# COx2/docker-nvidia-glx-desktop

Measured on AMD Instinct MI355X. Metric: encoded FPS + p50 end-to-end latency at 1080p60 H.264; concurrent sessions/node, higher is better.
Workload: dtype uint8 video (8-bit 4:2:0), H.264 Constrained Baseline

## Files before the change

csrc/bindings/module.cpp:

```cpp
#include <pybind11/numpy.h>
#include <pybind11/pybind11.h>
#include <pybind11/stl.h>

#include <cstring>

#include "../codec/h264_core.h"
#include "../codec/h264_encoder.h"
#include "../codec/vp8_encoder.h"
#include "../codec/hevc_encoder.h"
#include "../common/hip_check.h"
#include "../common/trace.h"
#include "../kernels/pixel.h"
#include "../runtime/session.h"

namespace py = pybind11;
using namespace mx;

void register_net(py::module& m);
void register_audio(py::module& m);
void register_rfb(py::module& m);

namespace {

template <class T>
T* as_ptr(uintptr_t p) {
    return reinterpret_cast<T*>(p);
}
hipStream_t as_stream(uintptr_t s) { return reinterpret_cast<hipStream_t>(s); }

py::bytes to_bytes(const std::vector<uint8_t>& v) {
    return py::bytes(reinterpret_cast<const char*>(v.data()), v.size());
}

struct PyBits {
    std::vector<uint32_t> words;
    h264::BitWriter w;
    PyBits() : words(4096) { w.init(words.data()); }
    py::tuple finish() {
        const uint32_t bits = w.bits;
        w.flush();
        std::vector<uint8_t> out;
        for (uint32_t i = 0; i < (bits + 7) / 8; ++i) out.push_back((uint8_t)(words[i / 4] >> (24 - 8 * (i % 4))));
        return py::make_tuple(to_bytes(out), bits);
    }
};

py::tuple cavlc_block_py(const std::vector<int>& coef, int nc) {
    PyBits b;
    int16_t c[16] = {0};
    const int n = (int)coef.size();
    if (n != 4 && n != 15 && n != 16) throw std::invalid_argument("block must have 4, 15 or 16 coefficients");
    for (int i = 0; i < n; ++i) c[i] = (int16_t)coef[i];
    h264::cavlc_block(b.w, c, n, nc);
    return b.finish();
}

py::array_t<int> fdct_py(py::array_t<int, py::array::c_style | py::array::forcecast> x) {
    if (x.size() != 16) throw std::invalid_argument("need 16 values");
    py::array_t<int> y(16);
    h264::fdct4x4(x.data(), y.mutable_data());
    return y;
}
py::array_t<int> idct_py(py::array_t<int, py::array::c_style | py::array::forcecast> x) {
    if (x.size() != 16) throw std::invalid_argument("need 16 values");
    py::array_t<int> y(16);
    h264::idct4x4(x.data(), y.mutable_data());
    return y;
}

py::array_t<uint8_t> copy_plane(const uint8_t* dev, int pitch, int w, int h) {
    py::array_t<uint8_t> out({h, w});
    HIP_CHECK(hipDeviceSynchronize());
    HIP_CHECK(hipMemcpy2D(out.mutable_data(), w, dev, pitch, w, h, hipMemcpyDeviceToHost));
    return out;
}

}

PYBIND11_MODULE(_native, m) {
    m.doc() = "mxdesk native runtime: HIP kernels (gfx950), H.264 encoder, session pipeline";

    m.def("device_count", []() {
        int n = 0;
        if (hipGetDeviceCount(&n) != hipSuccess) return 0;
        return n;
    });
    m.def("set_device", [](int d) { HIP_CHECK(hipSetDevice(d)); });
    m.def("device_name", [](int d) {
        hipDeviceProp_t p;
        HIP_CHECK(hipGetDeviceProperties(&p, d));
        return std::string(p.gcnArchName) + " / " + p.name;
    });
    m.def("synchronize", []() { HIP_CHECK(hipDeviceSynchronize()); });
    register_net(m);
    register_audio(m);
    register_rfb(m);
    m.def("now_us", &Session::now_us, "CLOCK_MONOTONIC microseconds (same clock as time.monotonic())");

    py::module h = m.def_submodule("h264", "H.264 building blocks (for tests)");
    h.def("hpel_planes", [](py::array_t<uint8_t, py::array::c_style> ref, int coded_w) {
        if (ref.ndim() != 2 || coded_w % 16 || ref.shape(0) % 16 || ref.shape(1) < coded_w)
            throw std::invalid_argument("ref must be (coded_h, pitch) with 16-aligned coded size");
        int hp = 0;
        auto planes = h264::hpel_planes_for_test(ref.data(), coded_w, (int)ref.shape(0), (int)ref.shape(1), &hp);
        const int rows = (int)ref.shape(0) + 2 * h264::kHpelPad;
        py::list out;
        for (auto& p : planes) {
            py::array_t<uint8_t> a({rows, hp});
            std::memcpy(a.mutable_data(), p.data(), p.size());
            out.append(a);
        }
        return out;
    });
    h.def("mc_luma_gpu", [](py::array_t<uint8_t, py::array::c_style> ref, int coded_w, int x4, int y4) {
        if (ref.ndim() != 2 || coded_w % 16 || ref.shape(0) % 16 || ref.shape(1) < coded_w)
            throw std::invalid_argument("ref must be (coded_h, pitch) with 16-aligned coded size");
        py::array_t<uint8_t> out({16, 16});
        h264::mc_luma_for_test(ref.data(), coded_w, (int)ref.shape(0), (int)ref.shape(1), x4, y4, out.mutable_data());
        return out;
    }, py::arg("ref"), py::arg("coded_w"), py::arg("x4"), py::arg("y4"),
          "16x16 luma prediction at quarter-sample position (x4, y4) by k_inter_encode's interpolation");
    h.def("cavlc_block", &cavlc_block_py, py::arg("coef"), py::arg("nc"));
    h.def("fdct4x4", &fdct_py);
    h.def("idct4x4", &idct_py);
    h.def("ue", [](uint32_t k) {
        PyBits b;
        h264::put_ue(b.w, k);
        return b.finish();
    });
    h.def("se", [](int v) {
        PyBits b;
        h264::put_se(b.w, v);
        return b.finish();
    });
    h.def("luma_qpel", [](py::array_t<uint8_t, py::array::c_style> plane, int x4, int y4) {
        if (plane.ndim() != 2) throw std::invalid_argument("2-D plane");
        const int H = (int)plane.shape(0), W = (int)plane.shape(1);
        return h264::luma_qpel(plane.data(), W, W, H, x4, y4);
    });
    h.def("level_for", &h264::pick_level);
    h.def("zero_sum_4x4", [](int qp) { return h264::zero_sum_4x4(qp); }, py::arg("qp"));
    h.def("zero_sum_chroma_dc", [](int qpc) { return h264::zero_sum_chroma_dc(qpc); }, py::arg("qpc"));
    h.def("chroma_qp", [](int qp, int offset) { return h264::chroma_qp(qp, offset); }, py::arg("qp"),
          py::arg("offset") = 0);
    h.def("quant4x4", [](py::array_t<int, py::array::c_style | py::array::forcecast> y, int qp, bool intra, int start) {
        if (y.size() != 16) throw std::invalid_argument("need 16 values");
        py::array_t<int> z(16);
        const int nz = h264::quant4x4(y.data(), z.mutable_data(), qp, intra, start);
        return py::make_tuple(z, nz);
    }, py::arg("y"), py::arg("qp"), py::arg("intra") = false, py::arg("start") = 0);
    h.def("quant_dc_chroma", [](py::array_t<int, py::array::c_style | py::array::forcecast> dc, int qpc, bool intra) {
        if (dc.size() != 4) throw std::invalid_argument("need 4 values");
        py::array_t<int> z(4);
        const int nz = h264::quant_dc_chroma(dc.data(), z.mutable_data(), qpc, intra);
        return py::make_tuple(z, nz);
    }, py::arg("dc"), py::arg("qpc"), py::arg("intra") = false);
    h.def("luma_block_inter", [](py::array_t<int, py::array::c_style | py::array::forcecast> res, int qp) {
        if (res.size() != 16) throw std::invalid_argument("need 16 values");
        py::array_t<int> z(16), rr(16);
        const int nz = h264::luma_block_inter(res.data(), qp, z.mutable_data(), rr.mutable_data());
        return py::make_tuple(z, rr, nz);
    }, py::arg("res"), py::arg("qp"), "inter luma block: residual (raster) -> levels (scan), reconstructed residual, nz");

    py::class_<h264::EncoderConfig>(m, "EncoderConfig")
        .def(py::init<>())
        .def_readwrite("width", &h264::EncoderConfig::width)
        .def_readwrite("height", &h264::EncoderConfig::height)
        .def_readwrite("fps", &h264::EncoderConfig::fps)
        .def_readwrite("bitrate_kbps", &h264::EncoderConfig::bitrate_kbps)
        .def_readwrite("qp", &h264::EncoderConfig::qp)
        .def_readwrite("qp_min", &h264::EncoderConfig::qp_min)
        .def_readwrite("qp_max", &h264::EncoderConfig::qp_max)
        .def_readwrite("keyint", &h264::EncoderConfig::keyint)
        .def_readwrite("search_range", &h264::EncoderConfig::search_range)
        .def_readwrite("scroll_range", &h264::EncoderConfig::scroll_range)
        .def_readwrite("me_coarse", &h264::EncoderConfig::me_coarse)
        .def_readwrite("intra4x4", &h264::EncoderConfig::intra4x4)
        .def_readwrite("subpel", &h264::EncoderConfig::subpel)
        .def_readwrite("chroma_qp_offset", &h264::EncoderConfig::chroma_qp_offset)
        .def_readwrite("pipeline_depth", &h264::EncoderConfig::pipeline_depth)
        .def_readwrite("aq", &h264::EncoderConfig::aq)
        .def_readwrite("intra_in_p", &h264::EncoderConfig::intra_in_p)
        .def_readwrite("vp8_bpred", &h264::EncoderConfig::vp8_bpred)
        .def_readwrite("vp8_intra", &h264::EncoderConfig::vp8_intra)
        .def_readwrite("mask_x0", &h264::EncoderConfig::mask_x0)
        .def_readwrite("mask_y0", &h264::EncoderConfig::mask_y0)
        .def_readwrite("mask_x1", &h264::EncoderConfig::mask_x1)
        .def_readwrite("mask_y1", &h264::EncoderConfig::mask_y1)
        .def_readwrite("deblock", &h264::EncoderConfig::deblock)
        .def_readwrite("partitions", &h264::EncoderConfig::partitions)
        .def_readwrite("tu_split", &h264::EncoderConfig::tu_split)
        .def_readwrite("hevc_slice_cost", &h264::EncoderConfig::hevc_slice_cost)
        .def_readwrite("hevc_wpp", &h264::EncoderConfig::hevc_wpp)
        .def_readwrite("hevc_wpp_rows", &h264::EncoderConfig::hevc_wpp_rows)
        .def_readwrite("sao", &h264::EncoderConfig::sao)
        .def_readwrite("hevc_chroma_keep", &h264::EncoderConfig::hevc_chroma_keep)
        .def_readwrite("hevc_intra_split", &h264::EncoderConfig::hevc_intra_split);

    py::class_<h264::FrameStats>(m, "FrameStats")
        .def_readonly("frame_index", &h264::FrameStats::frame_index)
        .def_readonly("idr", &h264::FrameStats::idr)
        .def_readonly("qp", &h264::FrameStats::qp)
        .def_readonly("bytes", &h264::FrameStats::bytes)
        .def_readonly("skipped_mbs", &h264::FrameStats::skipped_mbs)
        .def_readonly("encode_ms", &h264::FrameStats::encode_ms)
// ... 715 lines not shown
```

csrc/codec/h264_core.h:

```cpp
#pragma once
#include <hip/hip_runtime.h>
#include <stdint.h>

#include "h264_tables.h"

#define MXHD __host__ __device__ __forceinline__

namespace mx {
namespace h264 {

struct BitWriter {
    uint32_t* words;
    uint32_t nwords;
    uint64_t acc;
    int nacc;
    uint32_t bits;

    MXHD void init(uint32_t* w) {
        words = w;
        nwords = 0;
        acc = 0;
        nacc = 0;
        bits = 0;
    }
// ... 207 lines not shown
    if (nC < 8) return 2;
    return 3;
}

template <class W>
MXHD int cavlc_block(W& w, const int16_t* coef, int maxNum, int nC) {
    int total = 0, last = -1, t1 = 0;
    bool t1_open = true;
    for (int i = maxNum - 1; i >= 0; --i) {
        const int c = coef[i];
        if (c != 0) {
            if (last < 0) last = i;
            if (t1_open) {
                if ((c == 1 || c == -1) && t1 < 3) ++t1;
                else t1_open = false;
            }
            ++total;
        }
    }
    const int tab = nc_table(nC);
    if (total == 0) {
        w.put(kCoeffToken0[tab].code, kCoeffToken0[tab].len);
        return 0;
    }
    const Vlc ct = kCoeffToken[tab][total - 1][t1];
    w.put(ct.code, ct.len);
    int sl = (total > 10 && t1 < 3) ? 1 : 0;
    int k = 0;
    for (int i = last; i >= 0; --i) {
        const int l = coef[i];
        if (l == 0) continue;
        if (k < t1) {
            w.put(l < 0 ? 1u : 0u, 1);
            ++k;
            continue;
        }
        int code = l > 0 ? 2 * l - 2 : -2 * l - 1;
        if (k == t1 && t1 < 3) code -= 2;
        if (sl == 0) {
            if (code < 14) {
                w.put(1, code + 1);
            } else if (code < 30) {
                w.put(1, 15);
                w.put(code - 14, 4);
            } else {
                w.put(1, 16);
                w.put(code - 30, 12);
            }
        } else {
            if (code < (15 << sl)) {
                w.put(1, (code >> sl) + 1);
                w.put(code & ((1 << sl) - 1), sl);
            } else {
                w.put(1, 16);
                w.put(code - (15 << sl), 12);
            }
        }
        if (sl == 0) sl = 1;
        const int a = l < 0 ? -l : l;
        if (a > (3 << (sl - 1)) && sl < 6) ++sl;
        ++k;
    }
    const int total_zeros = last + 1 - total;
    if (total < maxNum) {
        const Vlc tz = (maxNum == 4) ? kTotalZerosDc[total - 1][total_zeros] : kTotalZeros[total - 1][total_zeros];
        w.put(tz.code, tz.len);
    }
    int zl = total_zeros;
    int i = last;
    for (int seen = 0; seen < total - 1 && zl > 0; ++seen) {
        int j = i - 1, rb = 0;
        while (coef[j] == 0) {
            ++rb;
            --j;
        }
        const Vlc v = kRunBefore[(zl > 7 ? 7 : zl) - 1][rb];
        w.put(v.code, v.len);
        zl -= rb;
        i = j;
    }
    return total;
}

struct SeqParams {
    int width, height;
    int mb_w, mb_h;
    int level_idc;
    int log2_max_frame_num;
    int fps_num, fps_den;
};

MXHD int pick_level(int mbs, int fps) {
    long mbps = (long)mbs * fps;
    if (mbs <= 1620 && mbps <= 40500) return 30;
    if (mbs <= 3600 && mbps <= 108000) return 31;
    if (mbs <= 5120 && mbps <= 216000) return 32;
    if (mbs <= 8192 && mbps <= 245760) return 40;
    if (mbs <= 8704 && mbps <= 522240) return 42;
    if (mbs <= 22080 && mbps <= 589824) return 50;
    if (mbs <= 36864 && mbps <= 983040) return 51;
    if (mbs <= 36864) return 52;
    if (mbs <= 139264 && mbps <= 4177920) return 60;
    if (mbs <= 139264 && mbps <= 8355840) return 61;
    return 62;
}

template <class W>
MXHD void write_sps(W& w, const SeqParams& p) {
    w.put(66, 8);
    w.put(0xC0, 8);
    w.put(p.level_idc, 8);
    put_ue(w, 0);
    put_ue(w, p.log2_max_frame_num - 4);
    put_ue(w, 2);
    put_ue(w, 1);
    w.put(0, 1);
    put_ue(w, p.mb_w - 1);
    put_ue(w, p.mb_h - 1);
    w.put(1, 1);
    w.put(1, 1);
    const int crop_r = (p.mb_w * 16 - p.width) / 2, crop_b = (p.mb_h * 16 - p.height) / 2;
    if (crop_r || crop_b) {
        w.put(1, 1);
        put_ue(w, 0);
        put_ue(w, crop_r);
        put_ue(w, 0);
        put_ue(w, crop_b);
    } else {
        w.put(0, 1);
    }
    w.put(1, 1);
    w.put(0, 1);
    w.put(0, 1);
    w.put(1, 1);
    w.put(5, 3);
    w.put(0, 1);
    w.put(1, 1);
    w.put(1, 8);
    w.put(1, 8);
    w.put(1, 8);
    w.put(0, 1);
    w.put(1, 1);
    w.put((uint32_t)p.fps_den, 32);
    w.put((uint32_t)(2 * p.fps_num), 32);
    w.put(0, 1);
    w.put(0, 1);
    w.put(0, 1);
    w.put(0, 1);
    w.put(1, 1);
    w.put(1, 1);
    put_ue(w, 0);
    put_ue(w, 0);
    put_ue(w, 16);
    put_ue(w, 16);
    put_ue(w, 0);
    put_ue(w, 1);
    w.put(1, 1);
    w.flush();
}

template <class W>
MXHD void write_pps(W& w, int init_qp, int chroma_qp_offset) {
    put_ue(w, 0);
    put_ue(w, 0);
    w.put(0, 1);
    w.put(0, 1);
// ... 177 lines not shown
```

csrc/codec/h264_kernels.hip:

```cpp
#include <hip/hip_runtime.h>

#include <cstddef>

#include "../common/hip_check.h"
#include "../common/wave.h"
#include "h264_core.h"
#include "h264_deblock.h"
#include "h264_gpu.h"
#include "h264_mb.h"

namespace mx {
namespace h264 {

namespace {

__device__ __forceinline__ uint32_t bswap32(uint32_t v) { return __builtin_bswap32(v); }

constexpr int kHpTW = 128, kHpTH = 16;
constexpr int kHpSW = kHpTW + 8;
__device__ __forceinline__ int byte_of(uint32_t w, int k) { return (int)((w >> (8 * k)) & 0xff); }
__device__ __forceinline__ uint32_t pack4(int a, int b, int c, int d) {
    const uint32_t lo = __builtin_amdgcn_perm((uint32_t)b, (uint32_t)a, 0x0c0c0400u);
    const uint32_t hi = __builtin_amdgcn_perm((uint32_t)d, (uint32_t)c, 0x0c0c0400u);
    return __builtin_amdgcn_perm(hi, lo, 0x05040100u);
// ... 2092 lines not shown
        intra_luma_mb(g, f, ls, m, mc, mbx, mby, av, lt, ldc, lane, s0);
        const int r = lane >> 2, c4 = (lane & 3) * 4;
        const uint32_t v = (uint32_t)lt[1 + r][1 + c4] | ((uint32_t)lt[1 + r][2 + c4] << 8) |
                           ((uint32_t)lt[1 + r][3 + c4] << 16) | ((uint32_t)lt[1 + r][4 + c4] << 24);
        *reinterpret_cast<uint32_t*>(fs->rec_y + (y0 + r) * g.pitch + x0 + c4) = v;
    } else {
        const int xc0 = mbx * 8, yc0 = mby * 8;
        if (lane < 32) {
            const int r = lane >> 2, c4 = (lane & 3) * 4;
            cs[lane] = *reinterpret_cast<const uint32_t*>(src_uv + (size_t)(yc0 + r) * g.pitch + mbx * 16 + c4);
        }
        if (lane < 16) {
            const int comp = lane >> 3, r = lane & 7;
            ct[comp][1 + r][0] = av.left ? fs->rec_uv[(yc0 + r) * g.pitch + 2 * (xc0 - 1) + comp] : 0;
        } else if (lane < 34) {
            const int k = lane - 16, comp = k / 9, cx = k - comp * 9;
            const bool ok = cx == 0 ? av.topleft : av.top;
            ct[comp][0][cx] = ok ? fs->rec_uv[(yc0 - 1) * g.pitch + 2 * (xc0 - 1 + cx) + comp] : 0;
        }
        wave_lds_sync();
        intra_chroma_mb(g, fs->chroma_qp_offset, f, cs, m, mc, mbx, mby, av, ct, cdc, lane, s0, s1);
        if (lane < 32) {
            const int r = lane >> 2, c2 = (lane & 3) * 2;
            const uint32_t v = (uint32_t)ct[0][1 + r][1 + c2] | ((uint32_t)ct[1][1 + r][1 + c2] << 8) |
                               ((uint32_t)ct[0][1 + r][2 + c2] << 16) | ((uint32_t)ct[1][1 + r][2 + c2] << 24);
            *reinterpret_cast<uint32_t*>(fs->rec_uv + (yc0 + r) * g.pitch + 2 * (xc0 + c2)) = v;
        }
    }
    unsigned long long a = s0, b = s1;
    for (int o = 32; o > 0; o >>= 1) {
        a += __shfl_xor(a, o, 64);
        b += __shfl_xor(b, o, 64);
    }
    __syncthreads();
    const int nmb = g.mb_w * g.mb_h;
    const int slot = mby;
    if (lane == 0) {
        if (wave == 0) {
            m.cbp = (uint8_t)((m.cbp & 15) | (m.cbp_c << 4));
            atomicAdd(&fs->sse_part[slot], a - mb_sse[mbi]);
            if (mb_unmasked(fs, mbx, mby)) atomicAdd(&fs->sse_part[3 * kSsePartStride + slot], a - mb_sse[mbi]);
        } else {
            atomicAdd(&fs->sse_part[kSsePartStride + slot], a - mb_sse[nmb + mbi]);
            atomicAdd(&fs->sse_part[2 * kSsePartStride + slot], b - mb_sse[2 * nmb + mbi]);
        }
    }
}

__global__ __launch_bounds__(128) void k_intra_p(Geometry g, const FrameState* __restrict__ fs,
                                                 const uint8_t* __restrict__ src_y, const uint8_t* __restrict__ src_uv,
                                                 MbInfo* __restrict__ mbs, int16_t* __restrict__ coef,
                                                 const int32_t* __restrict__ gain, const uint32_t* __restrict__ mb_sse,
                                                 const int* __restrict__ wave_prog, const int* __restrict__ cand) {
    const int ncand = wave_prog[1];
    for (int k = blockIdx.x; k < ncand; k += gridDim.x) intra_p_mb(g, fs, src_y, src_uv, mbs, coef, gain, mb_sse, cand[k]);
}

__device__ __forceinline__ uint32_t mask_bits(int n) { return n >= 32 ? 0xffffffffu : ((1u << n) - 1); }

template <class F>
__device__ __forceinline__ void overlap(uint32_t& acc, uint32_t W0, uint32_t s0, uint32_t len, F getbits) {
    const uint32_t lo = max(W0, s0), hi = min(W0 + 32, s0 + len);
    if (lo >= hi) return;
    const int n = (int)(hi - lo);
    const uint32_t bits = getbits(lo - s0, n) & mask_bits(n);
    acc |= bits << (W0 + 32 - hi);
}

constexpr int kRoleWords = 24;
__device__ __forceinline__ uint32_t role_get(const uint32_t* buf, uint32_t b, int n) {
    const uint32_t wi = b >> 5, sh = b & 31;
    const uint64_t hi = ((uint64_t)buf[wi] << 32) | (wi + 1 < (uint32_t)kRoleWords ? buf[wi + 1] : 0u);
    return (uint32_t)((hi << sh) >> (64 - n));
}

constexpr int kCavlcMbPerBlock = 8;
template <bool kQuad>
__global__ __launch_bounds__(256) void k_cavlc(Geometry g, const FrameState* __restrict__ fs, MbInfo* __restrict__ mbs,
                                               const int16_t* __restrict__ coef, uint32_t* __restrict__ slot,
                                               uint32_t* __restrict__ slot_bits) {
    static_assert(kNumRoles < 32, "the roles of one MB (plus the total slot) must fit a half-wave");
    __shared__ uint32_t rbuf[kCavlcMbPerBlock][kNumRoles][kRoleWords];
    __shared__ uint32_t roff[kCavlcMbPerBlock][kNumRoles + 1];
    __shared__ __attribute__((aligned(16))) int16_t cbuf[kCavlcMbPerBlock][kCoefStride];
    __shared__ MbInfo nbuf[kCavlcMbPerBlock][5];
    static_assert(sizeof(MbInfo) % 4 == 0, "MbInfo copied as dwords");
    const int hw = (threadIdx.x >> 5) & 1, lane = threadIdx.x & 31;
    const int wave = threadIdx.x >> 5;
    const int nmb = g.mb_w * g.mb_h;
    const int mbi = blockIdx.x * kCavlcMbPerBlock + wave;
    if (mbi >= nmb) return;
    const int mbx = mbi % g.mb_w, mby = mbi / g.mb_w;
    const Avail av = mb_avail(g, mbx, mby, fs->slice_rows);
    {
        const int src[5] = {mbi, mbi - 1, mbi - g.mb_w, mbi - g.mb_w + 1, mbi - g.mb_w - 1};
        const bool ok[5] = {true, av.left, av.top, av.topright, av.topleft};
        constexpr int kW = (int)(sizeof(MbInfo) / 4);
        for (int q = lane; q < 5 * kW; q += 32) {
            const int k = q / kW, d = q - k * kW;
            if (ok[k]) reinterpret_cast<uint32_t*>(&nbuf[wave][k])[d] = reinterpret_cast<const uint32_t*>(&mbs[src[k]])[d];
        }
        wave_lds_sync();
    }
    const MbNbrs nb{&nbuf[wave][0], &nbuf[wave][1], &nbuf[wave][2], &nbuf[wave][3], &nbuf[wave][4]};
    const MbInfo& m = nbuf[wave][0];
    const int16_t* mc = coef + (size_t)mbi * kCoefStride;

    int mvd[kQuad ? 8 : 4];
    const bool skip = decide_skip<kQuad>(nb, av, mvd);
    int dqp = 0;
    if (!skip && !fs->idr && carries_dqp(m)) {
        const int per_slice = fs->slice_rows * g.mb_w, first = (mbi / per_slice) * per_slice;
        int pred = fs->qp;
        bool found = false;
        constexpr int kPer = 16;
        for (int j0 = mbi - 1; j0 >= first && !found; j0 -= 32 * kPer) {
            int qv[kPer];
#pragma unroll
            for (int k = 0; k < kPer; ++k) {
                const int j = j0 - 32 * k - lane;
                qv[k] = -1;
                if (j >= first) {
                    const MbInfo& mj = mbs[j];
                    if (carries_dqp(mj)) qv[k] = mj.qp;
                }
            }
#pragma unroll
            for (int k = 0; k < kPer; ++k) {
                const unsigned long long bal = __ballot(qv[k] >= 0);
                const uint32_t hb = (uint32_t)(bal >> (32 * hw));
                const int q = __shfl(qv[k], hb ? (int)(__ffs(hb) - 1) : 0, 32);
                if (!found && hb) {
                    pred = q;
                    found = true;
                }
            }
        }
        dqp = qp_delta(m.qp, pred);
    }
    if (!skip) {
        const uint4* src = reinterpret_cast<const uint4*>(mc);
        uint4* dst = reinterpret_cast<uint4*>(cbuf[wave]);
        for (int q = lane; q < kCoefStride / 8; q += 32) dst[q] = src[q];
    }
    wave_lds_sync();
    uint32_t bits = 0;
    if (!skip && lane < kNumRoles) {
        BitWriter w;
        w.init(rbuf[wave][lane]);
        code_role<kQuad>(w, lane, g, fs->idr, nb, cbuf[wave], av, mvd, dqp);
        w.flush();
        bits = w.bits;
    }
    uint32_t incl = bits;
    incl += (uint32_t)__builtin_amdgcn_update_dpp(0, (int)incl, 0x111, 0xF, 0xF, false);
    incl += (uint32_t)__builtin_amdgcn_update_dpp(0, (int)incl, 0x112, 0xF, 0xF, false);
    incl += (uint32_t)__builtin_amdgcn_update_dpp(0, (int)incl, 0x114, 0xF, 0xF, false);
    incl += (uint32_t)__builtin_amdgcn_update_dpp(0, (int)incl, 0x118, 0xF, 0xF, false);
    incl += (uint32_t)__builtin_amdgcn_update_dpp(0, (int)incl, 0x142, 0xA, 0xF, false);
    const uint32_t total = __shfl(incl, 31, 32);
    if (lane < kNumRoles) roff[wave][lane] = incl - bits;
    if (lane == kNumRoles) roff[wave][kNumRoles] = total;
    wave_lds_sync();
    const bool fits = total <= kSlotWords * 32u;
    if (!skip && fits) {
        const uint32_t nwords = (total + 31) >> 5;
        uint32_t* dst = slot + (size_t)mbi * kSlotWords;
        for (uint32_t wi = lane; wi < nwords; wi += 32) {
            const uint32_t W0 = wi * 32;
            int r = 0;
            while (r < kNumRoles - 1 && roff[wave][r + 1] <= W0) ++r;
            uint32_t acc = 0;
            for (; r < kNumRoles; ++r) {
                const uint32_t o = roff[wave][r], len = roff[wave][r + 1] - o;
                if (o >= W0 + 32) break;
                if (len == 0) continue;
                overlap(acc, W0, o, len, [&](uint32_t x, int n) { return role_get(rbuf[wave][r], x, n); });
            }
            dst[wi] = acc;
        }
    }
    if (lane == 0) {
        slot_bits[mbi] = skip ? 0u : (fits ? total : 0xffffffffu);
        mbs[mbi].skip = skip ? 1 : 0;
    }
}

constexpr int kScanThreads = 256;
constexpr int kScanRowPer = 2;
constexpr int kScanMaxRows = 512;

__device__ __forceinline__ uint32_t blk_excl_sum(uint32_t v, uint32_t* wbuf, uint32_t* total) {
    return blk_excl_scan<kScanThreads, uint32_t>(v, 0u, [](uint32_t a, uint32_t b) { return a + b; }, wbuf, total);
}
__device__ __forceinline__ int blk_excl_max(int v, int init, int* wbuf, int* total) {
    return blk_excl_scan<kScanThreads, int>(v, init, [](int a, int b) { return max(a, b); }, wbuf, total);
}

__device__ __forceinline__ SliceParams slice_params(const FrameState* fs, int s, int mb_w) {
    return make_slice_params(s * fs->slice_rows * mb_w, fs->idr, fs->frame_num, fs->log2_max_frame_num,
                             fs->idr_pic_id, fs->qp - fs->pic_init_qp, fs->deblock_off);
}

template <bool kQuad>
__global__ __launch_bounds__(kScanThreads) void k_scan_rows(Geometry g, const FrameState* __restrict__ fs,
                                                            const uint32_t* __restrict__ slot_bits,
                                                            uint4* __restrict__ row_agg,
                                                            unsigned long long* __restrict__ row_sse,
                                                            const MbInfo* __restrict__ mbs, uint32_t* __restrict__ db_cnt,
                                                            const uint32_t* __restrict__ mb_sse) {
    __shared__ int wi[kScanThreads / 64];
    __shared__ uint32_t wu[kScanThreads / 64];
    const int t = threadIdx.x, r = blockIdx.x, base = r * g.mb_w;
    const bool idr = fs->idr != 0;
    const int nmb = g.mb_w * g.mb_h;
    const bool per_mb = !idr && fs->deblock_off;
    unsigned long long acc[4] = {0, 0, 0, 0};
    if (per_mb) {
        for (int j = t; j < g.mb_w; j += kScanThreads) {
            const uint32_t sy = mb_sse[base + j];
            acc[0] += sy;
            acc[1] += mb_sse[nmb + base + j];
            acc[2] += mb_sse[2 * nmb + base + j];
            acc[3] += mb_unmasked(fs, j, r) ? sy : 0u;
        }
    }
    if (t == 0 && (!per_mb || fs->intra_in_p))
        for (int c = 0; c < 4; ++c) acc[c] += fs->sse_part[c * kSsePartStride + r];
    uint32_t b[kScanRowPer];
    int last = -1, first = 0x7fffffff;
    uint32_t ncoded = 0, over = 0;
#pragma unroll
    for (int k = 0; k < kScanRowPer; ++k) {
// ... 501 lines not shown
```

csrc/codec/h264_mb.h:

```cpp
#pragma once
#include "h264_core.h"
#include "h264_gpu.h"
#include "h264_intra.h"

namespace mx {
namespace h264 {

constexpr int kNumRoles = 28;

struct Avail {
    bool left, top, topright, topleft;
};

MXHD Avail mb_avail(const Geometry& g, int mbx, int mby, int slice_rows) {
    Avail a;
    const bool top_same_slice = mby > 0 && (mby / slice_rows) == ((mby - 1) / slice_rows);
    a.left = mbx > 0;
    a.top = top_same_slice;
    a.topright = top_same_slice && mbx < g.mb_w - 1;
    a.topleft = top_same_slice && mbx > 0;
    return a;
}

MXHD int combine_nc(bool ha, int na, bool hb, int nb) {
// ... 73 lines not shown
            c = mv_nb_blk<kQuad>(nb.left, av.left, 3, 1);
            if (a.ref == 0) return a.mv;
        }
    } else {
        if (idx == 0) {
            a = mv_nb_blk<kQuad>(nb.left, av.left, 3, 0);
            b = mv_nb_blk<kQuad>(nb.top, av.top, 0, 3);
            c = av.top ? mv_nb_blk<kQuad>(nb.top, true, 2, 3) : mv_nb_blk<kQuad>(nb.topleft, av.topleft, 3, 3);
            if (a.ref == 0) return a.mv;
        } else {
            a = own;
            b = mv_nb_blk<kQuad>(nb.top, av.top, 2, 3);
            c = av.topright ? mv_nb_blk<kQuad>(nb.topright, true, 0, 3) : mv_nb_blk<kQuad>(nb.top, av.top, 1, 3);
            if (c.ref == 0) return c.mv;
        }
    }
    return predict_mv16x16(a, b, c);
}

MXHD Mv predict_mv_quad(const MbNbrs& nb, const Avail& av, int q) {
    auto own = [&](int k) {
        MvNb n;
        n.avail = true;
        n.ref = 0;
        n.mv = quad_mv(*nb.self, k);
        return n;
    };
    MvNb a, b, c;
    if (q == 0) {
        a = mv_nb_blk(nb.left, av.left, 3, 0);
        b = mv_nb_blk(nb.top, av.top, 0, 3);
        c = av.top ? mv_nb_blk(nb.top, true, 2, 3) : mv_nb_blk(nb.topleft, av.topleft, 3, 3);
    } else if (q == 1) {
        a = own(0);
        b = mv_nb_blk(nb.top, av.top, 2, 3);
        c = av.topright ? mv_nb_blk(nb.topright, true, 0, 3) : mv_nb_blk(nb.top, av.top, 1, 3);
    } else if (q == 2) {
        a = mv_nb_blk(nb.left, av.left, 3, 2);
        b = own(0);
        c = own(1);
    } else {
        a = own(2);
        b = own(1);
        c = own(0);
    }
    return predict_mv16x16(a, b, c);
}

template <bool kQuad = true>
MXHD bool decide_skip(const MbNbrs& nb, const Avail& av, int* mvd) {
    const MbInfo& m = *nb.self;
    mvd[0] = mvd[1] = mvd[2] = mvd[3] = 0;
    if (kQuad) mvd[4] = mvd[5] = mvd[6] = mvd[7] = 0;
    if (m.type != kMbP16x16) return false;
    if (kQuad && m.part == kPart8x8) {
        for (int q = 0; q < 4; ++q) {
            const Mv v = quad_mv(m, q), p = predict_mv_quad(nb, av, q);
            mvd[2 * q] = v.x - p.x;
            mvd[2 * q + 1] = v.y - p.y;
        }
        return false;
    }
    if (m.part != kPart16x16) {
        const Mv v0{m.pmv[0], m.pmv[1]}, v1{m.pmv[2], m.pmv[3]};
        const Mv p0 = predict_mv_part<kQuad>(nb, av, m.part, 0, v0);
        const Mv p1 = predict_mv_part<kQuad>(nb, av, m.part, 1, v0);
        mvd[0] = v0.x - p0.x;
        mvd[1] = v0.y - p0.y;
        mvd[2] = v1.x - p1.x;
        mvd[3] = v1.y - p1.y;
        return false;
    }
    const MvNb a = mv_nb_blk<kQuad>(nb.left, av.left, 3, 0);
    const MvNb b = mv_nb_blk<kQuad>(nb.top, av.top, 0, 3);
    MvNb c = mv_nb_blk<kQuad>(nb.topright, av.topright, 0, 3);
    if (!av.topright) c = mv_nb_blk<kQuad>(nb.topleft, av.topleft, 3, 3);
    const Mv pskip = predict_mv_skip(a, b, c);
    const Mv p = predict_mv16x16(a, b, c);
    mvd[0] = m.mvx - p.x;
    mvd[1] = m.mvy - p.y;
    return m.cbp == 0 && m.mvx == pskip.x && m.mvy == pskip.y;
}

template <bool kQuad = true, class W>
MXHD void code_role(W& w, int role, const Geometry& g, int idr, const MbNbrs& nb, const int16_t* mc,
                    const Avail& av, const int* mvd, int dqp = 0) {
    const MbInfo& m = *nb.self;
    const bool intra = m.type == kMbI16x16;
    const int cbp = m.cbp;
    const int cbp_l = cbp & 15, cbp_c = cbp >> 4;
    const MbInfo* ml = av.left ? nb.left : nullptr;
    const MbInfo* mt = av.top ? nb.top : nullptr;
    if (role == 0) {
        if (intra) {
            const int mbtype = 1 + m.i16_mode + 4 * cbp_c + (cbp_l ? 12 : 0);
            put_ue(w, (uint32_t)(idr ? mbtype : 5 + mbtype));
            put_ue(w, m.chroma_mode);
            put_se(w, dqp);
        } else if (m.type == kMbI4x4) {
            put_ue(w, idr ? 0u : 5u);
            for (int b = 0; b < 16; ++b) {
                const int bx = kBlkX[b], by = kBlkY[b];
                const bool ha = bx > 0 || av.left, hb = by > 0 || av.top;
                int ma = -1, mb = -1;
                if (bx > 0) ma = i4_get(m.i4, by * 4 + bx - 1);
                else if (ml && ml->type == kMbI4x4) ma = i4_get(ml->i4, by * 4 + 3);
                if (by > 0) mb = i4_get(m.i4, (by - 1) * 4 + bx);
                else if (mt && mt->type == kMbI4x4) mb = i4_get(mt->i4, 12 + bx);
                const int pm = i4_pred_mode(ma, mb, ha, hb);
                const int mode = i4_get(m.i4, by * 4 + bx);
                if (mode == pm) {
                    w.put(1, 1);
                } else {
                    w.put(0, 1);
                    w.put((uint32_t)(mode < pm ? mode : mode - 1), 3);
                }
            }
            put_ue(w, m.chroma_mode);
            put_ue(w, (uint32_t)cbp_to_codenum(cbp, true));
            if (cbp) put_se(w, dqp);
        } else {
            put_ue(w, m.part);
            if (kQuad && m.part == kPart8x8)
                for (int q = 0; q < 4; ++q) put_ue(w, 0u);
            put_se(w, mvd[0]);
            put_se(w, mvd[1]);
            if (m.part != kPart16x16) {
                put_se(w, mvd[2]);
                put_se(w, mvd[3]);
            }
            if (kQuad && m.part == kPart8x8)
                for (int i = 4; i < 8; ++i) put_se(w, mvd[i]);
            put_ue(w, (uint32_t)cbp_to_codenum(cbp, false));
            if (cbp) put_se(w, dqp);
        }
        return;
    }
    if (role == 1) {
        if (!intra) return;
        const int nc = combine_nc(av.left, ml ? ml->nz_luma[3] : 0, av.top, mt ? mt->nz_luma[12] : 0);
        cavlc_block(w, mc + kCoefLumaDc, 16, nc);
        return;
    }
    if (role <= 17) {
        const int b = role - 2;
        if (!(cbp_l & (1 << (b >> 2)))) return;
        const int bx = kBlkX[b], by = kBlkY[b];
        const bool ha = bx > 0 || av.left, hb = by > 0 || av.top;
        const int na = bx > 0 ? m.nz_luma[by * 4 + bx - 1] : (ml ? ml->nz_luma[by * 4 + 3] : 0);
        const int nb = by > 0 ? m.nz_luma[(by - 1) * 4 + bx] : (mt ? mt->nz_luma[12 + bx] : 0);
        const int nc = combine_nc(ha, na, hb, nb);
        if (intra) {
            cavlc_block(w, mc + kCoefLuma + b * 16 + 1, 15, nc);
        } else {
            cavlc_block(w, mc + kCoefLuma + b * 16, 16, nc);
        }
        return;
    }
    if (role <= 19) {
        if (!cbp_c) return;
        const int comp = role - 18;
        cavlc_block(w, mc + kCoefChromaDc + comp * 4, 4, -1);
        return;
    }
    if (role < kNumRoles) {
        if (cbp_c != 2) return;
        const int comp = (role - 20) >> 2, cb = (role - 20) & 3, bx = cb & 1, by = cb >> 1;
        const uint8_t* own = comp ? m.nz_cr : m.nz_cb;
        const uint8_t* lft = ml ? (comp ? ml->nz_cr : ml->nz_cb) : nullptr;
        const uint8_t* top = mt ? (comp ? mt->nz_cr : mt->nz_cb) : nullptr;
        const bool ha = bx > 0 || av.left, hb = by > 0 || av.top;
        const int na = bx > 0 ? own[by * 2] : (lft ? lft[by * 2 + 1] : 0);
        const int nb = by > 0 ? own[bx] : (top ? top[2 + bx] : 0);
        const int nc = combine_nc(ha, na, hb, nb);
        cavlc_block(w, mc + kCoefChromaAc + (comp * 4 + cb) * 16 + 1, 15, nc);
    }
}

MXHD int aq_mb_qp(int frame_qp, uint32_t sad, int aq) {
    if (!aq) return frame_qp;
    const int off = sad > 256u * 48 ? 12 : (sad > 256u * 32 ? 6 : 0);
    const int q = frame_qp + off;
    return q > 51 ? 51 : q;
}

MXHD int lambda_sse(int qp) {
    constexpr int tab[52] = {0,   0,   0,   0,   0,   0,   0,   0,   0,    0,    1,    1,    1,    1,
                             1,   2,   2,   3,   3,   4,   5,   7,   9,    11,   14,   17,   22,   27,
                             34,  43,  54,  69,  86,  109, 137, 173, 218,  274,  345,  435,  548,  691,
                             870, 1097, 1382, 1741, 2193, 2763, 3482, 4387, 5527, 6963};
    return tab[qp < 0 ? 0 : (qp > 51 ? 51 : qp)];
}
MXHD uint32_t block_bits_est(int nz) { return nz ? 2u + 6u * (uint32_t)nz : 0u; }
MXHD bool drop_residual(int aq, uint32_t lsad, int qp, long long d_pred, long long d_coded, uint32_t bits) {
    if (aq < 2 || lsad <= 256u * 32) return false;
    return d_pred - d_coded < (long long)lambda_sse(qp) * (long long)bits;
}

constexpr uint32_t kTsadChanging = 256u * 24, kTsadPersistent = 256u * 2;
constexpr int kAqChangingOffset = 6, kAqPersistentOffset = -6;
MXHD int aq_static_offset(int aq) { return kAqPersistentOffset - 3 * ((aq > 6 ? 6 : aq) - 3); }
enum TClass : int { kTcNormal = 0, kTcPersistent = 1, kTcChanging = 2, kTcStatic = 3 };
MXHD int temporal_class(uint32_t tsad, bool zero_mv) {
    return tsad > kTsadChanging ? kTcChanging
                                : (tsad == 0 && zero_mv ? kTcStatic : (tsad <= kTsadPersistent ? kTcPersistent : kTcNormal));
}
MXHD int aq3_mb_qp(int frame_qp, int tclass, int aq = 3) {
    const int q = frame_qp + (tclass == kTcChanging     ? kAqChangingOffset
                              : tclass == kTcStatic     ? aq_static_offset(aq)
                              : tclass == kTcPersistent ? kAqPersistentOffset
                                                        : 0);
    return q < 0 ? 0 : (q > 51 ? 51 : q);
}
MXHD int mb_qp_for(int frame_qp, uint32_t lsad, int tclass, int aq) {
    return aq >= 3 ? aq3_mb_qp(frame_qp, tclass, aq) : aq_mb_qp(frame_qp, lsad, aq);
}
MXHD bool drop_luma_for(int aq, uint32_t lsad, int tclass, int qp, long long d_pred, long long d_coded,
                        uint32_t bits) {
    if (aq >= 3)
        return tclass == kTcChanging && d_pred - d_coded < (long long)lambda_sse(qp) * (long long)bits;
    return drop_residual(aq, lsad, qp, d_pred, d_coded, bits);
}
MXHD bool drop_luma_possible(int aq, uint32_t lsad, int tclass) {
    return aq >= 3 ? tclass == kTcChanging : (aq >= 2 && lsad > 256u * 32);
}
MXHD bool drop_chroma_for(int aq, int tclass, bool luma_dropped) {
    return luma_dropped || (aq >= 3 && tclass == kTcChanging);
}

MXHD uint32_t inter_cost(uint32_t satd, int frame_qp, int mvx, int mvy) {
    return satd + (uint32_t)(lambda_sad(frame_qp) * (mvd_bits(mvx) + mvd_bits(mvy)));
}
template <bool kQuad = true>
MXHD uint32_t inter_cost_mb(uint32_t satd, int frame_qp, const MbInfo& m) {
    if (m.part == kPart16x16) return inter_cost(satd, frame_qp, m.mvx, m.mvy);
    if (kQuad && m.part == kPart8x8) {
        int bits = 0;
#pragma unroll
        for (int q = 0; q < 4; ++q) {
            const Mv v = quad_mv(m, q);
            bits += mvd_bits(v.x) + mvd_bits(v.y);
        }
        return satd + (uint32_t)(lambda_sad(frame_qp) * bits);
    }
    return satd + (uint32_t)(lambda_sad(frame_qp) *
                             (mvd_bits(m.pmv[0]) + mvd_bits(m.pmv[1]) + mvd_bits(m.pmv[2]) + mvd_bits(m.pmv[3])));
}

MXHD int idr_slice_rows(int mb_h) {
    const int ns = (mb_h + 3) / 4;
    return (mb_h + ns - 1) / ns;
}

MXHD int qp_delta(int qp, int pred) { return ((qp - pred + 26 + 52) % 52) - 26; }

MXHD SliceParams make_slice_params(int first_mb, int idr, int frame_num, int log2_max_frame_num, int idr_pic_id,
                                   int qp_delta, int deblock_off) {
    SliceParams sp;
// ... 116 lines not shown
```

Baseline: 13210.

## Encode CAVLC blocks from registers with LDS-staged VLC tables and faster QP prediction

Measured after the change: 12870. 0.974x the previous value.

```diff
diff --git a/csrc/bindings/module.cpp b/csrc/bindings/module.cpp
--- a/csrc/bindings/module.cpp
+++ b/csrc/bindings/module.cpp
@@ -52,6 +52,18 @@
     if (n != 4 && n != 15 && n != 16) throw std::invalid_argument("block must have 4, 15 or 16 coefficients");
     for (int i = 0; i < n; ++i) c[i] = (int16_t)coef[i];
     h264::cavlc_block(b.w, c, n, nc);
+    return b.finish();
+}
+
+py::tuple cavlc_block_regs_py(const std::vector<int>& coef, int nc, int dc) {
+    PyBits b;
+    alignas(16) int16_t c[16] = {0};
+    const int n = (int)coef.size();
+    if (n != 4 && n != 15 && n != 16) throw std::invalid_argument("block must have 4, 15 or 16 coefficients");
+    const int off = n == 15 ? 1 : 0;
+    c[0] = (int16_t)dc;
+    for (int i = 0; i < n; ++i) c[i + off] = (int16_t)coef[i];
+    h264::cavlc_block_regs(b.w, c, n, nc);
     return b.finish();
 }
 
@@ -121,6 +133,7 @@
     }, py::arg("ref"), py::arg("coded_w"), py::arg("x4"), py::arg("y4"),
           "16x16 luma prediction at quarter-sample position (x4, y4) by k_inter_encode's interpolation");
     h.def("cavlc_block", &cavlc_block_py, py::arg("coef"), py::arg("nc"));
+    h.def("cavlc_block_regs", &cavlc_block_regs_py, py::arg("coef"), py::arg("nc"), py::arg("dc") = 0);
     h.def("fdct4x4", &fdct_py);
     h.def("idct4x4", &idct_py);
     h.def("ue", [](uint32_t k) {
diff --git a/csrc/codec/h264_core.h b/csrc/codec/h264_core.h
--- a/csrc/codec/h264_core.h
+++ b/csrc/codec/h264_core.h
@@ -313,6 +313,142 @@
     return total;
 }
 
+struct CavlcTables {
+    Vlc coeff_token0[5];
+    Vlc coeff_token[5][16][4];
+    Vlc total_zeros[15][16];
+    Vlc total_zeros_dc[3][4];
+    Vlc run_before[7][15];
+};
+static_assert(sizeof(Vlc) == 4 && sizeof(CavlcTables) % 4 == 0, "CavlcTables copied as dwords");
+constexpr CavlcTables make_cavlc_tables() {
+    CavlcTables t{};
+    for (int a = 0; a < 5; ++a) {
+        t.coeff_token0[a] = kCoeffToken0[a];
+        for (int b = 0; b < 16; ++b)
+            for (int c = 0; c < 4; ++c) t.coeff_token[a][b][c] = kCoeffToken[a][b][c];
+    }
+    for (int a = 0; a < 15; ++a)
+        for (int b = 0; b < 16; ++b) t.total_zeros[a][b] = kTotalZeros[a][b];
+    for (int a = 0; a < 3; ++a)
+        for (int b = 0; b < 4; ++b) t.total_zeros_dc[a][b] = kTotalZerosDc[a][b];
+    for (int a = 0; a < 7; ++a)
+        for (int b = 0; b < 15; ++b) t.run_before[a][b] = kRunBefore[a][b];
+    return t;
+}
+constexpr CavlcTables kCavlcTables = make_cavlc_tables();
+
+struct CoefRegs {
+    uint32_t d0, d1, d2, d3, d4, d5, d6, d7;
+};
+MXHD int coef_at(const CoefRegs& r, int p) {
+    const int i = p >> 1;
+    const uint32_t a = (i & 1) ? r.d1 : r.d0, b = (i & 1) ? r.d3 : r.d2;
+    const uint32_t c = (i & 1) ? r.d5 : r.d4, d = (i & 1) ? r.d7 : r.d6;
+    const uint32_t ab = (i & 2) ? b : a, cd = (i & 2) ? d : c;
+    const uint32_t v = (i & 4) ? cd : ab;
+    return (int16_t)(v >> ((p & 1) * 16));
+}
+template <bool kOne>
+MXHD uint32_t coef_pair_mask(uint32_t v) {
+    const int lo = (int16_t)v, hi = (int16_t)(v >> 16);
+    if (kOne) return (uint32_t)(lo == 1 || lo == -1) | (uint32_t)(hi == 1 || hi == -1) << 1;
+    return (uint32_t)(lo != 0) | (uint32_t)(hi != 0) << 1;
+}
+template <bool kOne>
+MXHD uint32_t coef_mask(const CoefRegs& r) {
+    return coef_pair_mask<kOne>(r.d0) | coef_pair_mask<kOne>(r.d1) << 2 | coef_pair_mask<kOne>(r.d2) << 4 |
+           coef_pair_mask<kOne>(r.d3) << 6 | coef_pair_mask<kOne>(r.d4) << 8 | coef_pair_mask<kOne>(r.d5) << 10 |
+           coef_pair_mask<kOne>(r.d6) << 12 | coef_pair_mask<kOne>(r.d7) << 14;
+}
+
+template <class W>
+MXHD int cavlc_block_regs(W& w, const int16_t* blk, int maxNum, int nC, const CavlcTables& vt = kCavlcTables) {
+    CoefRegs r{0, 0, 0, 0, 0, 0, 0, 0};
+#if defined(__HIP_DEVICE_COMPILE__)
+    if (maxNum == 4) {
+        const uint2 v = *reinterpret_cast<const uint2*>(blk);
+        r.d0 = v.x, r.d1 = v.y;
+    } else {
+        const uint4 lo = reinterpret_cast<const uint4*>(blk)[0], hi = reinterpret_cast<const uint4*>(blk)[1];
+        r.d0 = lo.x, r.d1 = lo.y, r.d2 = lo.z, r.d3 = lo.w;
+        r.d4 = hi.x, r.d5 = hi.y, r.d6 = hi.z, r.d7 = hi.w;
+    }
+#else
+    auto pair = [&](int i) { return (uint32_t)(uint16_t)blk[2 * i] | ((uint32_t)(uint16_t)blk[2 * i + 1] << 16); };
+    r.d0 = pair(0), r.d1 = pair(1);
+    if (maxNum != 4) r.d2 = pair(2), r.d3 = pair(3), r.d4 = pair(4), r.d5 = pair(5), r.d6 = pair(6), r.d7 = pair(7);
+#endif
+    uint32_t nz = coef_mask<false>(r), one = coef_mask<true>(r);
+    const int off = maxNum == 15 ? 1 : 0;
+    nz >>= off;
+    one >>= off;
+    const int tab = nc_table(nC);
+    if (nz == 0) {
+        const Vlc c0 = vt.coeff_token0[tab];
+        w.put(c0.code, c0.len);
+        return 0;
+    }
+    const int total = __builtin_popcount(nz), last = ilog2_u32(nz);
+    const uint32_t big = nz & ~one;
+    const int above = __builtin_popcount(big ? nz >> (ilog2_u32(big) + 1) : nz);
+    const int t1 = above < 3 ? above : 3;
+    const Vlc ct = vt.coeff_token[tab][total - 1][t1];
+    w.put(ct.code, ct.len);
+    int sl = (total > 10 && t1 < 3) ? 1 : 0;
+    int k = 0;
+    for (uint32_t m = nz; m; ++k) {
+        const int p = ilog2_u32(m);
+        m ^= 1u << p;
+        const int l = coef_at(r, p + off);
+        if (k < t1) {
+            w.put(l < 0 ? 1u : 0u, 1);
+            continue;
+        }
+        int code = l > 0 ? 2 * l - 2 : -2 * l - 1;
+        if (k == t1 && t1 < 3) code -= 2;
+        if (sl == 0) {
+            if (code < 14) {
+                w.put(1, code + 1);
+            } else if (code < 30) {
+                w.put(1, 15);
+                w.put(code - 14, 4);
+            } else {
+                w.put(1, 16);
+                w.put(code - 30, 12);
+            }
+        } else {
+            if (code < (15 << sl)) {
+                w.put(1, (code >> sl) + 1);
+                w.put(code & ((1 << sl) - 1), sl);
+            } else {
+                w.put(1, 16);
+                w.put(code - (15 << sl), 12);
+            }
+        }
+        if (sl == 0) sl = 1;
+        const int a = l < 0 ? -l : l;
+        if (a > (3 << (sl - 1)) && sl < 6) ++sl;
+    }
+    const int total_zeros = last + 1 - total;
+    if (total < maxNum) {
+        const Vlc tz = (maxNum == 4) ? vt.total_zeros_dc[total - 1][total_zeros] : vt.total_zeros[total - 1][total_zeros];
+        w.put(tz.code, tz.len);
+    }
+    int zl = total_zeros;
+    uint32_t m = nz ^ (1u << last);
+    for (int p = last; m && zl > 0;) {
+        const int q = ilog2_u32(m);
+        m ^= 1u << q;
+        const int rb = p - q - 1;
+        const Vlc v = vt.run_before[(zl > 7 ? 7 : zl) - 1][rb];
+        w.put(v.code, v.len);
+        zl -= rb;
+        p = q;
+    }
+    return total;
+}
+
 struct SeqParams {
     int width, height;
     int mb_w, mb_h;
diff --git a/csrc/codec/h264_kernels.hip b/csrc/codec/h264_kernels.hip
--- a/csrc/codec/h264_kernels.hip
+++ b/csrc/codec/h264_kernels.hip
@@ -2198,9 +2198,12 @@
     static_assert(kNumRoles < 32, "the roles of one MB (plus the total slot) must fit a half-wave");
     __shared__ uint32_t rbuf[kCavlcMbPerBlock][kNumRoles][kRoleWords];
     __shared__ uint32_t roff[kCavlcMbPerBlock][kNumRoles + 1];
-    __shared__ __attribute__((aligned(16))) int16_t cbuf[kCavlcMbPerBlock][kCoefStride];
     __shared__ MbInfo nbuf[kCavlcMbPerBlock][5];
     static_assert(sizeof(MbInfo) % 4 == 0, "MbInfo copied as dwords");
+    __shared__ CavlcTables vlc;
+    for (int q = threadIdx.x; q < (int)(sizeof(CavlcTables) / 4); q += 256)
+        reinterpret_cast<uint32_t*>(&vlc)[q] = reinterpret_cast<const uint32_t*>(&kCavlcTables)[q];
+    __syncthreads();
     const int hw = (threadIdx.x >> 5) & 1, lane = threadIdx.x & 31;
     const int wave = threadIdx.x >> 5;
     const int nmb = g.mb_w * g.mb_h;
@@ -2229,8 +2232,24 @@
         const int per_slice = fs->slice_rows * g.mb_w, first = (mbi / per_slice) * per_slice;
         int pred = fs->qp;
         bool found = false;
+        {
+            static_assert(offsetof(MbInfo, type) == 4 && offsetof(MbInfo, cbp) == 5, "MbInfo layout");
+            const int j = mbi - 1 - lane;
+            int qn = -1;
+            if (j >= first) {
+                const uint32_t tc = reinterpret_cast<const uint32_t*>(&mbs[j])[1];
+                const int qj = mbs[j].qp;
+                if ((tc & 0xff) == kMbI16x16 || (tc & 0xff00) != 0) qn = qj;
+            }
+            const uint32_t hb = (uint32_t)(__ballot(qn >= 0) >> (32 * hw));
+            const int q = __shfl(qn, hb ? (int)(__ffs(hb) - 1) : 0, 32);
+            if (hb) {
+                pred = q;
+                found = true;
+            }
+        }
         constexpr int kPer = 16;
-        for (int j0 = mbi - 1; j0 >= first && !found; j0 -= 32 * kPer) {
+        for (int j0 = mbi - 33; j0 >= first && !found; j0 -= 32 * kPer) {
             int qv[kPer];
 #pragma unroll
             for (int k = 0; k < kPer; ++k) {
@@ -2254,17 +2273,11 @@
         }
         dqp = qp_delta(m.qp, pred);
     }
-    if (!skip) {
-        const uint4* src = reinterpret_cast<const uint4*>(mc);
-        uint4* dst = reinterpret_cast<uint4*>(cbuf[wave]);
-        for (int q = lane; q < kCoefStride / 8; q += 32) dst[q] = src[q];
-    }
-    wave_lds_sync();
     uint32_t bits = 0;
     if (!skip && lane < kNumRoles) {
         BitWriter w;
         w.init(rbuf[wave][lane]);
-        code_role<kQuad>(w, lane, g, fs->idr, nb, cbuf[wave], av, mvd, dqp);
+        code_role<kQuad>(w, lane, g, fs->idr, nb, mc, av, mvd, dqp, vlc);
         w.flush();
         bits = w.bits;
     }
diff --git a/csrc/codec/h264_mb.h b/csrc/codec/h264_mb.h
--- a/csrc/codec/h264_mb.h
+++ b/csrc/codec/h264_mb.h
@@ -179,9 +179,18 @@
     return m.cbp == 0 && m.mvx == pskip.x && m.mvy == pskip.y;
 }
 
+template <class W>
+MXHD int code_block(W& w, const int16_t* blk, int maxNum, int nc, const CavlcTables& vt) {
+#if defined(__HIP_DEVICE_COMPILE__)
+    return cavlc_block_regs(w, blk, maxNum, nc, vt);
+#else
+    return cavlc_block(w, blk + (maxNum == 15 ? 1 : 0), maxNum, nc);
+#endif
+}
+
 template <bool kQuad = true, class W>
 MXHD void code_role(W& w, int role, const Geometry& g, int idr, const MbNbrs& nb, const int16_t* mc,
-                    const Avail& av, const int* mvd, int dqp = 0) {
+                    const Avail& av, const int* mvd, int dqp = 0, const CavlcTables& vt = kCavlcTables) {
     const MbInfo& m = *nb.self;
     const bool intra = m.type == kMbI16x16;
     const int cbp = m.cbp;
@@ -236,7 +245,7 @@
     if (role == 1) {
         if (!intra) return;
         const int nc = combine_nc(av.left, ml ? ml->nz_luma[3] : 0, av.top, mt ? mt->nz_luma[12] : 0);
-        cavlc_block(w, mc + kCoefLumaDc, 16, nc);
+        code_block(w, mc + kCoefLumaDc, 16, nc, vt);
         return;
     }
     if (role <= 17) {
@@ -248,16 +257,16 @@
         const int nb = by > 0 ? m.nz_luma[(by - 1) * 4 + bx] : (mt ? mt->nz_luma[12 + bx] : 0);
         const int nc = combine_nc(ha, na, hb, nb);
         if (intra) {
-            cavlc_block(w, mc + kCoefLuma + b * 16 + 1, 15, nc);
+            code_block(w, mc + kCoefLuma + b * 16, 15, nc, vt);
         } else {
-            cavlc_block(w, mc + kCoefLuma + b * 16, 16, nc);
+            code_block(w, mc + kCoefLuma + b * 16, 16, nc, vt);
         }
         return;
     }
     if (role <= 19) {
         if (!cbp_c) return;
         const int comp = role - 18;
-        cavlc_block(w, mc + kCoefChromaDc + comp * 4, 4, -1);
+        code_block(w, mc + kCoefChromaDc + comp * 4, 4, -1, vt);
         return;
     }
     if (role < kNumRoles) {
@@ -270,7 +279,7 @@
         const int na = bx > 0 ? own[by * 2] : (lft ? lft[by * 2 + 1] : 0);
         const int nb = by > 0 ? own[bx] : (top ? top[2 + bx] : 0);
         const int nc = combine_nc(ha, na, hb, nb);
-        cavlc_block(w, mc + kCoefChromaAc + (comp * 4 + cb) * 16 + 1, 15, nc);
+        code_block(w, mc + kCoefChromaAc + (comp * 4 + cb) * 16, 15, nc, vt);
     }
 }
 
```
